# amazon-science/siam-mot

Hardware: AMD Instinct MI355X
Metric: frame-pairs/sec at 720p, 30 active tracks; EMM xcorr HBM GB/s vs peak (higher is better)
Workload: dtype f32 (towers and correlation: fp16x2 operands on MFMA, fp32 accumulate, fp32-equivalent error); 1 GPU; EMM tracker-head frame pair (EMM.forward + EMM.extract_cache) on DLA-34-FPN 720p FPN maps (net input 704x1280, C=128, 5 levels), 30 tracks, one stream per GPU; hot path only: backbone / RPN / box head / solver are outside the timed region; tracks=30, channels=128, rz=15, rx=30, feature_sets=8, feature_bytes_rotated=307281920

## Files before the change

siam-mot_amd/csrc/common.hip:

```cpp
#include "smot_common.h"
#include <mutex>
#include <vector>
#include "knobs.h"
#include <stdlib.h>
#include <string.h>

namespace smot {

static thread_local char g_err[512] = {0};

void set_error(const char* fmt, ...) {
    va_list ap;
    va_start(ap, fmt);
    vsnprintf(g_err, sizeof(g_err), fmt, ap);
    va_end(ap);
}

static thread_local int g_feat_type = SMOT_FEAT_F32;
int feat_type() { return g_feat_type & ~SMOT_FEAT_CHANNELS_LAST; }
bool channels_last() { return (g_feat_type & SMOT_FEAT_CHANNELS_LAST) != 0; }
FeatTypeScope::FeatTypeScope(int ft) : prev(g_feat_type) { g_feat_type = ft; }
FeatTypeScope::~FeatTypeScope() { g_feat_type = prev; }
int check_feat_type(int ft, const char* who) {
    const int et = ft & ~SMOT_FEAT_CHANNELS_LAST;
// ... 3 lines not shown
    return SMOT_ERR_BAD_ARG;
}

}

extern "C" int smot_abi_version(void) { return SMOT_ABI_VERSION; }

extern "C" int smot_build_info(void) {
#ifdef SMOT_DEBUG
    return 1;
#else
    return 0;
#endif
}

#ifdef SMOT_DEBUG
namespace smot {
namespace {
struct KnobName {
    const char* name;
    int Knobs::*field;
};
const KnobName kKnobNames[] = {
    {"SMOT_NO_FUSE", &Knobs::no_fuse},           {"SMOT_ROI_GENERIC", &Knobs::roi_generic},
    {"SMOT_TOWER_DIRECT", &Knobs::tower_direct}, {"SMOT_TOWER_WIDE", &Knobs::tower_wide},
    {"SMOT_DECODE_SPLIT", &Knobs::decode_split}, {"SMOT_XCORR_VARIANT", &Knobs::xcorr_variant},
    {"SMOT_DECODE_2PASS", &Knobs::decode_two_pass}, {"SMOT_FUSED_GEN", &Knobs::fused_gen},
    {"SMOT_TOWER_OCT", &Knobs::tower_oct},
    {"SMOT_TOWER_BF3", &Knobs::tower_bf3},
    {"SMOT_FUSED_ORDER", &Knobs::fused_order},   {"SMOT_NO_HINT", &Knobs::no_hint},
    {"SMOT_FUSED_ABL", &Knobs::fused_abl},       {"SMOT_ANY_ORDER", &Knobs::any_order},
    {"SMOT_WINO_ABL", &Knobs::wino_abl},
    {"SMOT_TOWER_ABL", &Knobs::tower_abl},
};
int parse_knob(const char* name, const char* v) {
    if (strcmp(name, "SMOT_XCORR_VARIANT") == 0) {
        static const char* const names[] = {"default", "wave", "patch", "pk", "one", "mfma", "fill", "compute"};
        for (int i = 0; i < 8; ++i)
            if (strcmp(v, names[i]) == 0) return i;
    }
    return atoi(v);
}
Knobs read_env() {
    Knobs k;
    for (const KnobName& kn : kKnobNames) {
        const char* v = getenv(kn.name);
        if (v != nullptr && v[0] != 0) k.*(kn.field) = parse_knob(kn.name, v);
    }
    return k;
}
}
Knobs& knobs_mut() {
    static Knobs k = read_env();
    return k;
}
namespace {
struct KnobInit {
    KnobInit() { (void)knobs_mut(); }
} g_knob_init;
}
}

extern "C" int smot_debug_set_knob(const char* name, const char* value) {
    using namespace smot;
    SMOT_REQUIRE(name && value, "debug_set_knob: null argument");
    for (const KnobName& kn : kKnobNames)
// ... 179 lines not shown
```

siam-mot_amd/csrc/knobs.h:

```cpp
#pragma once

namespace smot {

enum XcorrVariant { XV_DEFAULT = 0, XV_WAVE, XV_PATCH, XV_PK, XV_ONE, XV_MFMA, XV_FILL, XV_COMPUTE };

struct Knobs {
    int no_fuse = 0;
    int roi_generic = 0;
    int tower_direct = 0;
    int tower_wide = 0;
    int decode_split = 0;
    int xcorr_variant = 0;
    int decode_two_pass = 0;
    int fused_gen = 0;
    int fused_order = 0;
    int no_hint = 0;
    int tower_oct = 0;
    int tower_bf3 = 1;
    int any_order = 0;
    int fused_abl = 0;
    int wino_abl = 0;
    int tower_abl = 0;
};

#ifdef SMOT_DEBUG
Knobs& knobs_mut();
inline const Knobs& knobs() { return knobs_mut(); }
bool launch_xcorr_variant(int variant, const float* x, const float* z, float* out, int planes, hipStream_t st);
#else
inline constexpr Knobs knobs() { return Knobs{}; }
#endif

}
```

siam-mot_amd/csrc/sr_xcorr.hip:

```cpp
#include "roi_common.h"
#include "xcorr_patch2.h"
#include "xcorr_patch1.h"
#include "xcorr_f16x2.h"
#include "knobs.h"
#include <type_traits>
namespace smot { int launch_plane_absmax(const float* resp, int planes, int hw, float* pm, hipStream_t st); }

namespace smot {

constexpr int FX_CH = 8;

struct SrOut {
    float* sr;
    float pad, half_e, two_e, min_wh;
    long long* trace;
    int abl;
    const int* n_valid;
    int order;
    float* hint_out;
    const float* hint_in;
    int hint_extra;
    int plan_pad[SMOT_MAX_LEVELS];
    float* plane_max;
};
// ... 380 lines not shown
    constexpr bool BATCHED = true;
    constexpr int NCH = FX_CH;
    constexpr bool P2 = false;
    constexpr bool NHWC = true;
#include "sr_xcorr_fused9_body.h"
}

}


namespace smot {
constexpr int FX_ORDER_DEFAULT = 1;
static inline int fused_order() {
    const int k = knobs().fused_order;
    return k == 0 ? FX_ORDER_DEFAULT : (k == 4 ? 0 : k);
}
static inline bool order_hint_rois(int N, bool consumer) {
    if (knobs().fused_gen == 2 || knobs().no_hint >= (consumer ? 1 : 2)) return false;
    return N >= 2 && N <= 256 && fused_order() == 1;
}
template <int RX, bool XCORR, int MM>
static void launch_fused_half(dim3 grid, hipStream_t st, const LevelParams& P, int C, const float* rois, const float* boxes,
                              const float* z, float* resp, float* out, int32_t* levels_out, const SrOut& S,
                              const ImageRows* I) {
    SMOT_HALF_TYPES(
        if (I != nullptr) {
            SMOT_LAUNCH((sr_xcorr_fused9_half_batched_kernel<FT, RX, 15, 2, XCORR, MM>), grid, dim3(512), 0, st, P, C, rois,
                        boxes, z, resp, out, levels_out, S, *I);
        } else {
            SMOT_LAUNCH((sr_xcorr_fused9_half_kernel<FT, RX, 15, 2, XCORR, MM>), grid, dim3(512), 0, st, P, C, rois, boxes, z,
                        resp, out, levels_out, S);
        })
}
static inline bool half_maps() { return feat_type() != SMOT_FEAT_F32; }

template <int RX, bool XCORR, int MM>
static void launch_fused_nhwc(dim3 grid, hipStream_t st, const LevelParams& P, int C, const float* rois, const float* boxes,
                              const float* z, float* resp, float* out, int32_t* levels_out, const SrOut& S,
                              const ImageRows* I) {
    ImageRows one;
    if (I == nullptr) {
        one.num_images = 1;
        one.row_start[0] = 0;
        for (int b = 1; b <= SMOT_MAX_IMAGES; ++b) one.row_start[b] = (int)grid.x;
        I = &one;
    }
    if (feat_type() == SMOT_FEAT_F32) {
        SMOT_LAUNCH((sr_xcorr_fused9_nhwc_kernel<float, RX, 15, 2, XCORR, MM>), grid, dim3(512), 0, st, P, C, rois, boxes, z,
                    resp, out, levels_out, S, *I);
    } else {
        SMOT_HALF_TYPES(SMOT_LAUNCH((sr_xcorr_fused9_nhwc_kernel<FT, RX, 15, 2, XCORR, MM>), grid, dim3(512), 0, st, P, C,
                                    rois, boxes, z, resp, out, levels_out, S, *I))
    }
}
static void launch_pool_nhwc(int out_size, dim3 grid, hipStream_t st, const LevelParams& P, int C, const float* rois,
                             const float* boxes, float* out, int32_t* levels_out, const SrOut& S, const ImageRows* I) {
    if (out_size == 30) launch_fused_nhwc<30, false, 0>(grid, st, P, C, rois, boxes, nullptr, nullptr, out, levels_out, S, I);
    else if (out_size == 7) launch_fused_nhwc<7, false, 0>(grid, st, P, C, rois, boxes, nullptr, nullptr, out, levels_out, S, I);
    else launch_fused_nhwc<15, false, 0>(grid, st, P, C, rois, boxes, nullptr, nullptr, out, levels_out, S, I);
}

template <int RX, bool XCORR>
static void launch_fused(dim3 grid, hipStream_t st, const LevelParams& P, int C, const float* rois, const float* boxes,
                         const float* z, float* resp, float* out, int32_t* levels_out, const SrOut& S) {
    if (channels_last()) {
        launch_fused_nhwc<RX, XCORR, (RX == 30 && XCORR) ? 1 : 0>(grid, st, P, C, rois, boxes, z, resp, out, levels_out, S, nullptr);
// ... 6 lines not shown
#ifdef SMOT_DEBUG
    if (knobs().fused_gen == 2 && S.n_valid == nullptr) {
        hipLaunchKernelGGL((sr_xcorr_fused8_kernel<RX, 15, 2, XCORR>), grid, dim3(512), 0, st, P, C, rois, boxes, z, resp,
                           out, levels_out, S);
        return;
    }
#endif
    if constexpr (RX == 30 && XCORR) {
#ifdef SMOT_DEBUG
        if (knobs().fused_abl == 8 || knobs().fused_abl == 9) {
            SMOT_LAUNCH((sr_xcorr_fused9_kernel<RX, 15, 2, XCORR>), grid, dim3(512), knobs().fused_abl == 9 ? 26000 : 0, st, P, C, rois,
                        boxes, z, resp, out, levels_out, S);
            return;
        }
#endif
#ifdef SMOT_DEBUG
        if (knobs().fused_abl == 10) {
            SMOT_LAUNCH((sr_xcorr_fused9_kernel<RX, 15, 2, XCORR, FX_CH, false, 2>), grid, dim3(512), 0, st, P, C, rois, boxes, z,
                        resp, out, levels_out, S);
            return;
        }
#endif
        SMOT_LAUNCH((sr_xcorr_fused9_kernel<RX, 15, 2, XCORR, FX_CH, false, 1>), grid, dim3(512), 0, st, P, C, rois, boxes, z,
                    resp, out, levels_out, S);
    } else {
        SMOT_LAUNCH((sr_xcorr_fused9_kernel<RX, 15, 2, XCORR>), grid, dim3(512), 0, st, P, C, rois, boxes, z, resp, out,
                    levels_out, S);
    }
}

int launch_roi_pool_separable(const LevelParams& P, int C, const float* rois, const float* level_boxes, int R,
                              int out_size, float* out, int32_t* levels_out, hipStream_t st) {
    dim3 grid(R, (C + FX_CH - 1) / FX_CH);
    SrOut none = {nullptr, 0.f, 0.f, 0.f, 0.f, g_trace, 0, nullptr, fused_order(), nullptr, nullptr, 0};
    if (channels_last()) {
        launch_pool_nhwc(out_size, grid, st, P, C, rois, level_boxes, out, levels_out, none, nullptr);
    } else if (out_size == 30) {
        launch_fused<30, false>(grid, st, P, C, rois, level_boxes, nullptr, nullptr, out, levels_out, none);
    } else if (out_size == 7 && half_maps()) {
        launch_fused_half<7, false, 0>(grid, st, P, C, rois, level_boxes, nullptr, nullptr, out, levels_out, none, nullptr);
    } else if (out_size == 7) {
        SMOT_LAUNCH((sr_xcorr_fused9_kernel<7, 15, 2, false>), grid, dim3(512), 0, st, P, C, rois, level_boxes,
                    (const float*)nullptr, (float*)nullptr, out, levels_out, none);
    } else {
        launch_fused<15, false>(grid, st, P, C, rois, level_boxes, nullptr, nullptr, out, levels_out, none);
    }
    return check_launch("roi_pool_separable");
}

int launch_extract_cache(const float* const* feats, const int* heights, const int* widths, const float* scales,
                         int num_levels, int C, const float* boxes, int N, int rz, float pad_pixels, float half_e,
                         float two_e, float min_wh, float* templates, float* sr, const int* n_valid, float* order_hint,
                         hipStream_t st, int hint_extra_rows) {
    LevelParams P;
    const int rc = fill_level_params(&P, feats, heights, widths, nullptr, scales, num_levels, "emm_extract_cache", C);
    if (rc) return rc;
    SMOT_REQUIRE(boxes && templates && sr, "emm_extract_cache: null pointer");
    if (!order_hint_rois(N, false) || rz != 15) order_hint = nullptr;
    SMOT_REQUIRE(order_hint == nullptr || ((((uintptr_t)order_hint) & 31) == 0 && (((uintptr_t)boxes) & 15) == 0),
                 "emm_extract_cache: the order hint must be 32-byte aligned (and the boxes 16-byte aligned)");
    dim3 grid(N, (C + FX_CH - 1) / FX_CH + (order_hint != nullptr ? 1 : 0));
    SrOut S = {sr, pad_pixels, half_e, two_e, min_wh, g_trace, 0, n_valid, fused_order(), order_hint, nullptr,
               n_valid != nullptr ? hint_extra_rows : 0};
    for (int l = 0; l < num_levels && l < SMOT_MAX_LEVELS; ++l) S.plan_pad[l] = (int)(pad_pixels * scales[l]);
    if (channels_last()) {
        launch_pool_nhwc(rz, grid, st, P, C, boxes, boxes, templates, nullptr, S, nullptr);
    } else if (rz == 7 && half_maps()) {
        launch_fused_half<7, false, 0>(grid, st, P, C, boxes, boxes, nullptr, nullptr, templates, nullptr, S, nullptr);
    } else if (rz == 7) {
        SMOT_LAUNCH((sr_xcorr_fused9_kernel<7, 15, 2, false>), grid, dim3(512), 0, st, P, C, boxes, boxes, (const float*)nullptr,
                    (float*)nullptr, templates, (int32_t*)nullptr, S);
    } else {
        launch_fused<15, false>(grid, st, P, C, boxes, boxes, nullptr, nullptr, templates, nullptr, S);
    }
    return check_launch("emm_extract_cache");
}

int launch_roi_pool_separable_batched(const LevelParams& P, int C, const float* rois, const float* level_boxes, int R,
                                      int out_size, float* out, hipStream_t st, const ImageRows& I) {
    dim3 grid(R, (C + FX_CH - 1) / FX_CH);
    SrOut none = {nullptr, 0.f, 0.f, 0.f, 0.f, g_trace, 0, nullptr, fused_order(), nullptr, nullptr, 0};
    if (channels_last()) {
        launch_pool_nhwc(out_size, grid, st, P, C, rois, level_boxes, out, nullptr, none, &I);
    } else if (half_maps()) {
        if (out_size == 30) launch_fused_half<30, false, 0>(grid, st, P, C, rois, level_boxes, nullptr, nullptr, out, nullptr, none, &I);
        else if (out_size == 7) launch_fused_half<7, false, 0>(grid, st, P, C, rois, level_boxes, nullptr, nullptr, out, nullptr, none, &I);
        else launch_fused_half<15, false, 0>(grid, st, P, C, rois, level_boxes, nullptr, nullptr, out, nullptr, none, &I);
    } else if (out_size == 30) {
        SMOT_LAUNCH((sr_xcorr_fused9_batched_kernel<30, 15, 2, false>), grid, dim3(512), 0, st, P, C, rois, level_boxes,
                    (const float*)nullptr, (float*)nullptr, out, (int32_t*)nullptr, none, I);
    } else if (out_size == 7) {
        SMOT_LAUNCH((sr_xcorr_fused9_batched_kernel<7, 15, 2, false>), grid, dim3(512), 0, st, P, C, rois, level_boxes,
                    (const float*)nullptr, (float*)nullptr, out, (int32_t*)nullptr, none, I);
    } else {
        SMOT_LAUNCH((sr_xcorr_fused9_batched_kernel<15, 15, 2, false>), grid, dim3(512), 0, st, P, C, rois, level_boxes,
                    (const float*)nullptr, (float*)nullptr, out, (int32_t*)nullptr, none, I);
    }
    return check_launch("roi_pool_separable_batched");
}

int launch_extract_cache_batched(const float* const* feats, const int* heights, const int* widths, const float* scales,
                                 int num_levels, int C, const float* boxes, int N, int rz, float pad_pixels, float half_e,
                                 float two_e, float min_wh, float* templates, float* sr, float* order_hint, hipStream_t st,
                                 const ImageRows& I) {
    LevelParams P;
    const int rc = fill_level_params(&P, feats, heights, widths, nullptr, scales, num_levels, "emm_extract_cache_batched", C);
    if (rc) return rc;
    SMOT_REQUIRE(boxes && templates && sr, "emm_extract_cache_batched: null pointer");
    if (!order_hint_rois(N, false) || rz != 15) order_hint = nullptr;
    SMOT_REQUIRE(order_hint == nullptr || ((((uintptr_t)order_hint) & 31) == 0 && (((uintptr_t)boxes) & 15) == 0),
                 "emm_extract_cache_batched: the order hint must be 32-byte aligned (and the boxes 16-byte aligned)");
    dim3 grid(N, (C + FX_CH - 1) / FX_CH + (order_hint != nullptr ? 1 : 0));
    SrOut S = {sr, pad_pixels, half_e, two_e, min_wh, g_trace, 0, nullptr, fused_order(), order_hint, nullptr, 0};
    for (int l = 0; l < num_levels && l < SMOT_MAX_LEVELS; ++l) S.plan_pad[l] = (int)(pad_pixels * scales[l]);
    if (channels_last()) {
        launch_pool_nhwc(rz, grid, st, P, C, boxes, boxes, templates, nullptr, S, &I);
    } else if (half_maps()) {
        if (rz == 7) launch_fused_half<7, false, 0>(grid, st, P, C, boxes, boxes, nullptr, nullptr, templates, nullptr, S, &I);
        else launch_fused_half<15, false, 0>(grid, st, P, C, boxes, boxes, nullptr, nullptr, templates, nullptr, S, &I);
    } else if (rz == 7) {
        SMOT_LAUNCH((sr_xcorr_fused9_batched_kernel<7, 15, 2, false>), grid, dim3(512), 0, st, P, C, boxes, boxes,
                    (const float*)nullptr, (float*)nullptr, templates, (int32_t*)nullptr, S, I);
    } else {
        SMOT_LAUNCH((sr_xcorr_fused9_batched_kernel<15, 15, 2, false>), grid, dim3(512), 0, st, P, C, boxes, boxes,
                    (const float*)nullptr, (float*)nullptr, templates, (int32_t*)nullptr, S, I);
    }
    return check_launch("emm_extract_cache_batched");
}

int sr_xcorr_fused_batched_impl(const float* const* feats, const int* heights, const int* widths, const int* pad_cells,
                                const float* scales, int num_levels, int C, const float* boxes, const float* sr,
                                const float* templates, int N, float* resp, const float* order_hint, hipStream_t st,
                                const int** hint_status, float* plane_max, const ImageRows& I) {
    LevelParams P;
    const int rc = fill_level_params(&P, feats, heights, widths, pad_cells, scales, num_levels, "sr_xcorr_fused_batched", C);
    if (rc) return rc;
    if (!order_hint_rois(N, true)) order_hint = nullptr;
    if (hint_status != nullptr)
        *hint_status = order_hint != nullptr ? reinterpret_cast<const int*>(order_hint) + HINT_STATUS : nullptr;
    SMOT_REQUIRE(order_hint == nullptr || (((uintptr_t)order_hint) & 31) == 0,
                 "sr_xcorr_fused_batched: the order hint must be 32-byte aligned");
    dim3 grid(N, (C + FX_CH - 1) / FX_CH);
    SrOut none = {nullptr, 0.f, 0.f, 0.f, 0.f, g_trace, 0, nullptr, fused_order(), nullptr, order_hint, 0};
    none.plane_max = plane_max;
    timer_mark(0, 0, st);
    if (channels_last())
// ... 137 lines not shown
```

siam-mot_amd/csrc/sr_xcorr_fused9_body.h:

```cpp
    constexpr int HO = XCORR ? RX - RZ + 1 : 16;
    constexpr int NS = RX * G;
    constexpr int XS = P2 ? XP2_XS : (MM == 2 ? XL_XS : XP1_XS), XP = P2 ? XP2_XP : (MM == 2 ? 30 * XL_XS : 32 * XP1_XS), ZS = XP1_ZS,
                  ZP = MM == 1 ? XH_TZ_FLOATS : (MM == 2 ? XL_TZ_FLOATS : RZ * XP1_ZS);
    static_assert(MM == 0 || (XCORR && !P2 && RX == 30 && RZ == 15), "the matrix-pipe correlation is the 30 / 15 head's");
    static_assert(MM != 2 || ((XP * 4) % 128 == 0 && ((2 * XP + 2 * ZP) * 4) % 128 == 0), "lean layout: 128-byte aligned plane images");
    constexpr int RH = (RX + 1) / 2;
    static_assert((!XCORR || RX - RZ + 1 == 16) && RX <= 32 && G == 2 && RX * XS <= XP && 2 * RH * G <= 64,
                  "specialised for pooled sizes <= 32, g = 2 (and the 30/15/16 correlation geometry)");
    __shared__ __attribute__((aligned(128))) float sm[(NCH / 2) * (2 * XP + 2 * ZP)];
    __shared__ __attribute__((aligned(16))) int4 tab[2][64 + 2 * RH * G];
    __shared__ int wbound[4];

    const int tid = threadIdx.x;
    const int lane = tid & 63;
    const int wave = __builtin_amdgcn_readfirstlane(tid >> 6);
    const long long t_start = S.trace ? (long long)__builtin_amdgcn_s_memtime() : 0ll;
    const int ka_h = P.H[0], ka_w = P.W[0], ka_p = P.pad[0];
    const float ka_s = P.scale[0];
    const unsigned long long ka_f = reinterpret_cast<unsigned long long>(P.feat[0]);
#define SMOT_KA_USE() asm volatile("" ::"s"(ka_h), "s"(ka_w), "s"(ka_p), "s"(ka_s), "s"(ka_f))
    int ka_i[6] = {0, 0, 0, 0, 0, 0};
    if constexpr (BATCHED) {
        ka_i[0] = I.num_images;
#pragma unroll
        for (int k = 1; k < 6; ++k) ka_i[k] = I.row_start[min(16 * k - 1, SMOT_MAX_IMAGES)];
    }
#ifdef SMOT_DEBUG
    if (S.abl >= 100 && (int)(blockIdx.y * gridDim.x + blockIdx.x) >= 256) {
        for (int d = 0; d < S.abl - 100; ++d) __builtin_amdgcn_s_sleep(8);
    }
#endif
    int n_assigned, cg_assigned, lvl_assigned = 0;
    float4 roi_assigned = make_float4(0.f, 0.f, 0.f, 0.f);
    int grid_row = blockIdx.y, grid_rows = gridDim.y;
    if constexpr (!XCORR) {
        if (S.hint_out != nullptr) {
            if (grid_row == 0) {
                fx_write_hint<30, G>(P, boxes, S, gridDim.x, blockIdx.x, wave, lane);
                return;
            }
            grid_row -= 1;
            grid_rows -= 1;
        }
    }
// ... 64 lines not shown
        S.sr[n * 4 + 2] = o.z;
        S.sr[n * 4 + 3] = o.w;
    }
    const int H = P.H[lvl], W = P.W[lvl], pad = P.pad[lvl];
    const float scale = P.scale[lvl];
    const float x1 = mul_rn(roi[0], scale), y1 = mul_rn(roi[1], scale);
    const float x2 = mul_rn(roi[2], scale), y2 = mul_rn(roi[3], scale);
    const float bin_h = div_rn(fmaxf(sub_rn(y2, y1), 1.0f), (float)RX);
    const float bin_w = div_rn(fmaxf(sub_rn(x2, x1), 1.0f), (float)RX);
    FX_TRACE(6)
    constexpr int nplanes = NCH;
    const int c0 = cgrp * NCH;
    const bool owns = (wave < nplanes && c0 + wave < C);
    const int plane = n * C + c0 + wave;
    constexpr int NZ = XCORR ? (RZ * RZ + 63) / 64 : 1;
    float zreg[NZ];
    float zq[4] = {0.0f, 0.0f, 0.0f, 0.0f}, isz = 1.0f;
    if constexpr (MM != 0) {
        if (owns) xh_template_load(z + (size_t)plane * (RZ * RZ), lane, zq);
    } else if (XCORR && owns) {
        const float* __restrict__ zg = z + (size_t)plane * (RZ * RZ);
#pragma unroll
        for (int t = 0; t < NZ; ++t) zreg[t] = zg[min(lane + 64 * t, RZ * RZ - 1)];
    }

    const bool hent = XCORR && RX == 30 && k_assigned >= 0 && g8[4] == pad && g8[5] == H && g8[6] == W &&
                      g8[7] == __float_as_int(scale);
    const int hb[4] = {g8[0], g8[1], g8[2], g8[3]};
    const bool fast = !NHWC && MM == 1 && hent && hb[3] - hb[2] + 1 <= 64
#ifdef SMOT_DEBUG
                      && S.abl != 3 && S.abl != 12
#endif
        ;
    if (fast) {
    } else if (wave < 2 && hent) {
        tab[wave][lane] = tab_early;
        if (lane < 2 * RH * G) tab[wave][64 + lane] = make_int4(0, 0, 0, 0);
    } else if (wave < 2) {
        int lo = 0, hi = 0;
        float wl = 0.0f, wh = 0.0f;
        if (lane < NS) {
            if (wave == 0) {
                axis_sample(y1, bin_h, G, lane, H, pad, &lo, &hi, &wl, &wh);
            } else {
                axis_sample(x1, bin_w, G, lane, W, pad, &lo, &hi, &wl, &wh);
            }
        }
        int mn = 0x7fffffff, mx = -1;
        const unsigned long long m = __ballot(wl != 0.0f || wh != 0.0f);
        if (m != 0ull) {
            mn = __builtin_amdgcn_readlane((wl != 0.0f) ? lo : hi, __ffsll((long long)m) - 1);
            mx = __builtin_amdgcn_readlane((wh != 0.0f) ? hi : lo, 63 - __clzll((long long)m));
        }
        const int rl = (wl != 0.0f) ? lo : mn, rh = (wh != 0.0f) ? hi : mn;
        int4 e;
        if (wave == 0) {
            e.x = (int)((unsigned)(rl * W) * 4u);
            e.y = (int)((unsigned)(rh * W) * 4u);
        } else {
            e.x = (wl != 0.0f) ? lo - mn : 0;
            e.y = (wh != 0.0f) ? hi - mn : 0;
        }
        e.z = __float_as_int(wl);
        e.w = __float_as_int(wh);
        tab[wave][lane] = e;
        if (lane < 2 * RH * G) tab[wave][64 + lane] = make_int4(0, 0, 0, 0);
        if (lane == 0) {
            wbound[2 * wave] = mn;
            wbound[2 * wave + 1] = mx;
        }
    }
    FX_TRACE(7)
    if (!fast) __syncthreads();
    const int ymin = hent ? hb[0] : wbound[0], ymax = hent ? hb[1] : wbound[1];
    const int xmin = hent ? hb[2] : wbound[2], xmax = hent ? hb[3] : wbound[3];
    if (ymax < ymin || xmax < xmin) {
        if (owns) {
            if (XCORR) {
                for (int e = lane; e < HO * HO; e += 64) resp[(size_t)plane * HO * HO + e] = 0.0f;
                if (S.plane_max != nullptr && lane == 0) S.plane_max[plane] = 0.0f;
            }
            if (x_debug != nullptr)
                for (int e = lane; e < RX * RX; e += 64) x_debug[(size_t)plane * RX * RX + e] = 0.0f;
        }
        return;
    }
    const int ww = xmax - xmin + 1;
    FX_TRACE(1)

    if constexpr (MM != 0) {
    } else if (XCORR && owns) {
        float* zs = sm + (wave >> 1) * (2 * XP + 2 * ZP) + 2 * XP + (wave & 1) * ZP;
#pragma unroll
        for (int t = 0; t < NZ; ++t) {
            const int e = lane + 64 * t;
            if (e < RZ * RZ) {
                const int u = e / RZ;
                zs[u * ZS + (e - u * RZ)] = zreg[t];
            }
        }
    }
    FX_TRACE(2)

    const FT* __restrict__ fbase = reinterpret_cast<const FT*>(P.feat[lvl]);
    if constexpr (BATCHED) fbase += (size_t)img * ((size_t)C * H * W);
    const unsigned plane_bytes = (unsigned)(H * W) * (unsigned)sizeof(FT);
    constexpr int ROW_SHIFT = sizeof(FT) == 2 ? 1 : 0;
    auto pool = [&](auto pair_tag, auto chunk_tag, auto x2_tag, auto rows_tag) {
        constexpr bool PAIR = decltype(pair_tag)::value;
        constexpr bool CHUNKED = decltype(chunk_tag)::value;
        constexpr bool X2 = decltype(x2_tag)::value;
        constexpr int ROWS = decltype(rows_tag)::value;
        constexpr int NV = X2 ? 2 : 1;
        static_assert(!X2 || (PAIR && !CHUNKED), "two columns per lane is a form of the plane-pair mode");
        const int half = PAIR ? (lane >> 5) : 0;
        const int col = PAIR ? (lane & 31) : lane;
        const int pw = col < RX ? col : 0;
        const int pl0 = PAIR ? 2 * (wave >> 1) : wave;
        const bool has0 = (c0 + pl0 < C);
        const bool has1 = PAIR && (c0 + pl0 + 1 < C);
        if (!has0) return;
        const bool mine = PAIR ? (half == 0 || has1) : true;
        const unsigned lane_plane = (PAIR && half == 1 && has1) ? plane_bytes : 0u;
        float* xdst = sm + ((pl0 + half) >> 1) * (2 * XP + 2 * ZP) + ((pl0 + half) & 1) * XP;
        const FT* pbase = fbase + (size_t)(c0 + pl0) * H * W;
        unsigned long long pa = reinterpret_cast<unsigned long long>(pbase);
        const unsigned pa_lo = __builtin_amdgcn_readfirstlane((unsigned)pa);
        const unsigned pa_hi = __builtin_amdgcn_readfirstlane((unsigned)(pa >> 32));
        const auto rsrc = __builtin_amdgcn_make_buffer_rsrc(
            reinterpret_cast<void*>(((unsigned long long)pa_hi << 32) | pa_lo), 0, 0x7fffffff, 0x00020000);
        int sxl[G], sxh[G];
        float hxw[G], lxw[G];
#pragma unroll
        for (int ix = 0; ix < G; ++ix) {
            const int4 e = fast ? xe_early[ix] : tab[1][pw * G + ix];
            sxl[ix] = e.x;
            sxh[ix] = e.y;
            hxw[ix] = __int_as_float(e.z);
            lxw[ix] = __int_as_float(e.w);
        }
        const int row0 = PAIR ? (wave & 1) * RH : 0;
        const int nrows = PAIR ? RH : RX;
        const int nchunk = CHUNKED ? (ww + 63) >> 6 : 1;
        if constexpr (X2 && MM == 1) {
            constexpr int GR = (ROWS + 1) / 2, SW = 64;
            static_assert(RH % ROWS == 0 && GR * SW <= ROWS * XS, "full batches; staging fits a batch's own rows");
            const int wcol = min(2 * col, ww - 2);
            const unsigned voff = (unsigned)(xmin + wcol) * (unsigned)sizeof(FT) + lane_plane;
            typename fx_pair<FT>::type vl[ROWS][G], vh[ROWS][G];
            int4 ye = fast ? ye_early : tab[0][min(lane + row0 * G, 63 + 2 * RH * G)];
            ye.x = (int)((unsigned)ye.x >> ROW_SHIFT);
            ye.y = (int)((unsigned)ye.y >> ROW_SHIFT);
            int yoff = 0;
#define SMOT_FX_ISSUE()                                                                                             \
            _Pragma("unroll") for (int b = 0; b < ROWS; ++b)                                                        \
                _Pragma("unroll") for (int iy = 0; iy < G; ++iy) {                                                  \
                    vl[b][iy] = fx_load2<FT>(rsrc, voff, __builtin_amdgcn_readlane(ye.x, yoff + b * G + iy));         \
                    vh[b][iy] = fx_load2<FT>(rsrc, voff, __builtin_amdgcn_readlane(ye.y, yoff + b * G + iy));         \
                }
            SMOT_FX_ISSUE()
            __builtin_amdgcn_sched_barrier(0);
            if (owns) {
                unsigned char* tzw = reinterpret_cast<unsigned char*>(sm + (wave >> 1) * (2 * XP + 2 * ZP) + 2 * XP + (wave & 1) * ZP);
                isz = xh_template_store(zq, tzw, lane);
            }
            __builtin_amdgcn_sched_barrier(0);
#pragma unroll 1
            for (int r0 = row0; r0 < row0 + nrows; r0 += ROWS) {
                const float wl = __int_as_float(ye.z), wh = __int_as_float(ye.w);
                float cs[ROWS][NV];
#pragma unroll
                for (int b = 0; b < ROWS; ++b)
// ... 27 lines not shown
                    for (int b = g0; b < g0 + GR && b < ROWS; ++b)
#pragma unroll
                        for (int k = 0; k < NV; ++k) stage[(b - g0) * SW + wcol + k] = cs[b][k];
                    float p[GR][G][2];
#pragma unroll
                    for (int b = g0; b < g0 + GR && b < ROWS; ++b)
#pragma unroll
                        for (int ix = 0; ix < G; ++ix) {
                            p[b - g0][ix][0] = stage[(b - g0) * SW + sxl[ix]];
                            p[b - g0][ix][1] = stage[(b - g0) * SW + sxh[ix]];
                        }
                    __builtin_amdgcn_sched_barrier(0);
#pragma unroll
                    for (int b = g0; b < g0 + GR && b < ROWS; ++b)
#pragma unroll
                        for (int ix = 0; ix < G; ++ix) {
                            acc[b] = fmaf(hxw[ix], p[b - g0][ix][0], ix == 0 ? 0.0f : acc[b]);
                            acc[b] = fmaf(lxw[ix], p[b - g0][ix][1], acc[b]);
                        }
                    __builtin_amdgcn_sched_barrier(0);
                }
#pragma unroll
                for (int b = 0; b < ROWS; ++b) {
                    const int ph = r0 + b;
                    if (col < RX && ph < row0 + nrows && ph < RX && mine) xdst[ph * XS + col] = acc[b] * (1.0f / (float)(G * G));
                }
            }
#undef SMOT_FX_ISSUE
            return;
        }
#pragma unroll 1
        for (int r0 = row0; r0 < row0 + nrows; r0 += ROWS) {
            const int4 ye = (fast && PAIR && !CHUNKED) ? ye_early : tab[0][min(lane + r0 * G, 63 + 2 * RH * G)];
            const unsigned ol = (unsigned)ye.x >> ROW_SHIFT, oh = (unsigned)ye.y >> ROW_SHIFT;
            const float wl = __int_as_float(ye.z), wh = __int_as_float(ye.w);
            float acc[ROWS];
            if (CHUNKED) {
#pragma unroll
                for (int b = 0; b < ROWS; ++b) acc[b] = 0.0f;
            }
#pragma unroll 1
            for (int ch = 0; ch < nchunk; ++ch) {
                const int cbase = ch << 6;
                const int wcol = CHUNKED ? min(cbase + col, ww - 1) : (X2 ? min(2 * col, ww - 2) : min(col, ww - 1));
                const unsigned voff = (unsigned)(xmin + wcol) * (unsigned)sizeof(FT) + lane_plane;
                float v[ROWS][G][2][NV];
#pragma unroll
                for (int b = 0; b < ROWS; ++b)
#pragma unroll
                    for (int iy = 0; iy < G; ++iy) {
                        const int e = b * G + iy;
                        if constexpr (X2) {
                            const auto l2 = fx_load2<FT>(rsrc, voff, __builtin_amdgcn_readlane((int)ol, e));
                            const auto h2 = fx_load2<FT>(rsrc, voff, __builtin_amdgcn_readlane((int)oh, e));
                            v[b][iy][0][0] = fx_pair_elem<FT>(l2, 0);
                            v[b][iy][0][NV - 1] = fx_pair_elem<FT>(l2, 1);
                            v[b][iy][1][0] = fx_pair_elem<FT>(h2, 0);
                            v[b][iy][1][NV - 1] = fx_pair_elem<FT>(h2, 1);
                        } else {
                            v[b][iy][0][0] = fx_load1<FT>(rsrc, voff, __builtin_amdgcn_readlane((int)ol, e));
                            v[b][iy][1][0] = fx_load1<FT>(rsrc, voff, __builtin_amdgcn_readlane((int)oh, e));
                        }
                    }
                __builtin_amdgcn_sched_barrier(0);
                if constexpr (MM != 0) {
                    if (r0 == row0 && ch == 0 && owns) {
                        unsigned char* tzw = reinterpret_cast<unsigned char*>(sm + (wave >> 1) * (2 * XP + 2 * ZP) + 2 * XP + (wave & 1) * ZP);
                        isz = MM == 2 ? xl_template_store(zq, tzw, lane) : xh_template_store(zq, tzw, lane);
                    }
                    __builtin_amdgcn_sched_barrier(0);
                }
                float cs[ROWS][NV];
#pragma unroll
                for (int b = 0; b < ROWS; ++b)
#pragma unroll
                    for (int k = 0; k < NV; ++k) {
                        float c_ = 0.0f;
#pragma unroll
                        for (int iy = 0; iy < G; ++iy) {
                            const int e = b * G + iy;
                            c_ = fmaf(rl_f(wl, e), v[b][iy][0][k], c_);
                            c_ = fmaf(rl_f(wh, e), v[b][iy][1][k], c_);
                        }
                        cs[b][k] = c_;
                    }
                __builtin_amdgcn_sched_barrier(0);
                constexpr int GR = ((P2 || MM == 2) && X2) ? 3 : (ROWS + 1) / 2;
                if constexpr (!CHUNKED) {
                    constexpr int SW = (X2 || !PAIR) ? 64 : 32;
                    static_assert(GR * SW <= (RH - (RH / ROWS) * ROWS == 0 ? ROWS : RH - (RH / ROWS) * ROWS) * XS,
                                  "staging fits the image rows of the wave's LAST batch");
                    float* stage = xdst + r0 * XS;
#pragma unroll
                    for (int g0 = 0; g0 < ROWS; g0 += GR) {
#pragma unroll
                        for (int b = g0; b < g0 + GR && b < ROWS; ++b)
#pragma unroll
                            for (int k = 0; k < NV; ++k) stage[(b - g0) * SW + wcol + k] = cs[b][k];
                        float p[GR][G][2];
#pragma unroll
                        for (int b = g0; b < g0 + GR && b < ROWS; ++b)
#pragma unroll
                            for (int ix = 0; ix < G; ++ix) {
                                p[b - g0][ix][0] = stage[(b - g0) * SW + sxl[ix]];
                                p[b - g0][ix][1] = stage[(b - g0) * SW + sxh[ix]];
                            }
                        __builtin_amdgcn_sched_barrier(0);
#pragma unroll
                        for (int b = g0; b < g0 + GR && b < ROWS; ++b)
#pragma unroll
                            for (int ix = 0; ix < G; ++ix) {
                                acc[b] = fmaf(hxw[ix], p[b - g0][ix][0], ix == 0 ? 0.0f : acc[b]);
                                acc[b] = fmaf(lxw[ix], p[b - g0][ix][1], acc[b]);
// ... 5 lines not shown
                    bool inl[G], inh[G];
#pragma unroll
                    for (int ix = 0; ix < G; ++ix) {
                        const int tl = sxl[ix] - cbase, th = sxh[ix] - cbase;
                        inl[ix] = (unsigned)tl < 64u;
                        inh[ix] = (unsigned)th < 64u;
                        al[ix] = (tl & 63) << 2;
                        ah[ix] = (th & 63) << 2;
                    }
#pragma unroll
                    for (int g0 = 0; g0 < ROWS; g0 += GR) {
                        float p[GR][G][2];
#pragma unroll
                        for (int b = g0; b < g0 + GR && b < ROWS; ++b)
#pragma unroll
                            for (int ix = 0; ix < G; ++ix) {
                                p[b - g0][ix][0] = __int_as_float(__builtin_amdgcn_ds_bpermute(al[ix], __float_as_int(cs[b][0])));
                                p[b - g0][ix][1] = __int_as_float(__builtin_amdgcn_ds_bpermute(ah[ix], __float_as_int(cs[b][0])));
                            }
                        __builtin_amdgcn_sched_barrier(0);
#pragma unroll
                        for (int b = g0; b < g0 + GR && b < ROWS; ++b)
#pragma unroll
                            for (int ix = 0; ix < G; ++ix) {
                                acc[b] = inl[ix] ? fmaf(hxw[ix], p[b - g0][ix][0], acc[b]) : acc[b];
                                acc[b] = inh[ix] ? fmaf(lxw[ix], p[b - g0][ix][1], acc[b]) : acc[b];
                            }
                    }
                }
            }
#pragma unroll
            for (int b = 0; b < ROWS; ++b) {
                const int ph = r0 + b;
                if (col < RX && ph < row0 + nrows && ph < RX && mine) xdst[ph * XS + col] = acc[b] * (1.0f / (float)(G * G));
            }
        }
    };
    if constexpr (NHWC) {
#include "sr_pool_nhwc_stage.h"
    } else
    if (ww <= 32) {
        pool(std::true_type{}, std::false_type{}, std::false_type{}, std::integral_constant<int, RH>{});
#ifdef SMOT_DEBUG
    } else if (ww <= 64 && S.abl == 3 && MM != 2) {
        if constexpr (MM != 2) pool(std::false_type{}, std::false_type{}, std::false_type{}, std::integral_constant<int, RH>{});
#endif
    } else if (ww <= 64) {
        if constexpr (MM == 1) pool(std::true_type{}, std::false_type{}, std::true_type{}, std::integral_constant<int, RH / 3>{});
        else pool(std::true_type{}, std::false_type{}, std::true_type{}, std::integral_constant<int, (RH + 1) / 2>{});
    } else {
        pool(std::false_type{}, std::true_type{}, std::false_type{}, std::integral_constant<int, (RH + 2) / 3>{});
    }
    FX_TRACE(3)
    __syncthreads();
    if (x_debug != nullptr && owns) {
        const float* xs = sm + (wave >> 1) * (2 * XP + 2 * ZP) + (wave & 1) * XP;
        for (int e = lane; e < RX * RX; e += 64) {
            const int r = e / RX;
            x_debug[(size_t)plane * RX * RX + e] = xs[r * XS + (e - r * RX)];
        }
    }
    if constexpr (XCORR) {
#ifdef SMOT_DEBUG
        if (S.abl == 2) return;
#endif
        if constexpr (P2) {
            if (wave < nplanes / 2 && c0 + 2 * wave < C) {
                const float* xs2 = sm + wave * (2 * XP + 2 * ZP);
                xcorr_patch2_compute<RX, RZ, 0>(xs2, xs2 + 2 * XP, lane, resp, n * C + c0 + 2 * wave, n * C + min(C, c0 + NCH));
            }
        } else if (owns) {
            float* xs1 = sm + (wave >> 1) * (2 * XP + 2 * ZP) + (wave & 1) * XP;
            const float* zs1 = sm + (wave >> 1) * (2 * XP + 2 * ZP) + 2 * XP + (wave & 1) * ZP;
            if constexpr (MM == 1) xh_correlate<RX, RZ>(xs1, reinterpret_cast<const unsigned char*>(zs1), isz, lane, resp, plane, S.plane_max);
            else if constexpr (MM == 2) xl_correlate<RX, RZ>(xs1, reinterpret_cast<const unsigned char*>(zs1), isz, lane, resp, plane, S.plane_max);
            else xcorr_patch1_compute<RX, RZ, true>(xs1, zs1, lane, resp, plane, S.plane_max);
        }
    }
    FX_TRACE(4)
#undef FX_TRACE
```

siam-mot_amd/ops.py:

```python
import contextlib
import ctypes
import struct
import weakref
import os

import torch

_HERE = os.path.dirname(os.path.abspath(__file__))
LIB_PATH = os.path.join(_HERE, "csrc", "libsmot_emm.so")
DEBUG_LIB_PATH = os.path.join(_HERE, "csrc", "libsmot_emm_debug.so")
ABI_VERSION = 14
UP_SCALE = 16


_lib = None
_c_float_p = ctypes.POINTER(ctypes.c_float)
_vp = ctypes.c_void_p
_i = ctypes.c_int
_f = ctypes.c_float

_SIGNATURES = {
    "smot_abi_version": (ctypes.c_int, []),
    "smot_build_info": (ctypes.c_int, []),
    "smot_last_error": (ctypes.c_char_p, []),
# ... 82 lines not shown
    "smot_debug_sr_xcorr_fused_hint_fwd": (ctypes.c_int, [_vp, _vp, _vp, _vp, _vp, _i, _i, _vp, _vp, _vp, _i, _vp, _vp, _vp]),
}
DEBUG_EXPORTED_SYMBOLS = tuple(_DEBUG_SIGNATURES.keys())


def load_library(path=None):
    global _lib
    if _lib is not None and path is None:
        return _lib
    path = path or LIB_PATH
    if not os.path.exists(path):
        raise RuntimeError(
            "siammot_amd: HIP library %s not found — build it with `python siam-mot_amd/build.py` "
            "(hipcc --offload-arch=gfx950).  There is no CPU fallback." % path)
    _lib = _open(path, _SIGNATURES)
    return _lib


def _open(path, signatures):
    lib = ctypes.CDLL(path)
    for name, (res, args) in signatures.items():
        fn = getattr(lib, name)
        fn.restype = res
        fn.argtypes = args
    if lib.smot_abi_version() != ABI_VERSION:
        raise RuntimeError("siammot_amd: %s has ABI %d, host layer expects %d"
                           % (path, lib.smot_abi_version(), ABI_VERSION))
    return lib


_KNOB_DEFAULTS = {"SMOT_NO_FUSE": "0", "SMOT_ROI_GENERIC": "0", "SMOT_TOWER_DIRECT": "0", "SMOT_TOWER_WIDE": "0",
                  "SMOT_DECODE_SPLIT": "0", "SMOT_XCORR_VARIANT": "default", "SMOT_DECODE_2PASS": "0",
                  "SMOT_FUSED_GEN": "0", "SMOT_TOWER_OCT": "0", "SMOT_TOWER_BF3": "1", "SMOT_FUSED_ORDER": "0", "SMOT_NO_HINT": "0", "SMOT_FUSED_ABL": "0",
                  "SMOT_ANY_ORDER": "0",
                  "SMOT_WINO_ABL": "0",
                  "SMOT_TOWER_ABL": "0"}


@contextlib.contextmanager
def debug_library(**knobs):
    global _lib
    if not os.path.exists(DEBUG_LIB_PATH):
        raise RuntimeError("siammot_amd: measurement library %s not built (python siam-mot_amd/build.py)" % DEBUG_LIB_PATH)
    load_library()
    dbg = _open(DEBUG_LIB_PATH, dict(_SIGNATURES, **_DEBUG_SIGNATURES))
    if not (dbg.smot_build_info() & 1):
        raise RuntimeError("siammot_amd: %s is not a measurement build" % DEBUG_LIB_PATH)
    prev, _lib = _lib, dbg

    def set_all(values):
        for k, v in values.items():
            if dbg.smot_debug_set_knob(k.encode(), str(v).encode()) != 0:
                raise RuntimeError("siammot_amd: " + dbg.smot_last_error().decode("utf-8", "replace"))
    try:
        set_all(_KNOB_DEFAULTS)
        set_all(knobs)
        _hint_floats.clear()
        yield dbg
    finally:
        set_all(_KNOB_DEFAULTS)
        _lib = prev
        _hint_floats.clear()


def _check(rc, what):
    if rc != 0:
        msg = _lib.smot_last_error().decode("utf-8", "replace")
# ... 1290 lines not shown
```

Baseline: 18400 frame-pairs/s.

## Add lean pool-only extraction path with register tables and direct global stores

For the non-xcorr, NCHW pooling instantiation (template extraction), each wave now computes its y/x sampling entries in registers and reads them by lane through bpermute and readlane. This replaces the shared-memory table build, its barrier, and the reduction of bounds through shared memory. Pooled outputs are written straight to global memory instead of being staged in LDS and copied out after a __syncthreads. The aim is to cut barriers and LDS traffic in the short extraction kernel. The cost is scattered, stride-RX global stores and more cross-lane shuffles; a debug knob keeps the old path, and a trace script is added.

```diff
diff --git a/measure/debug/extract_trace.py b/measure/debug/extract_trace.py
--- /dev/null
+++ b/measure/debug/extract_trace.py
@@ -0,0 +1,51 @@
+import json, os, sys
+import numpy as np, torch
+sys.path.insert(0, os.path.join(os.path.dirname(__file__), "..", ".."))
+import bench
+import siammot_amd.ops as ops
+dev = torch.device("cuda:0")
+ops.load_library()
+scales = (0.25, 0.125, 0.0625, 0.03125)
+args = sys.argv[1:]
+split = args.index("--") if "--" in args else len(args)
+counts = [int(a) for a in args[:split]] or [30]
+variants = [dict(kv.split("=") for kv in v.split(",")) for v in args[split + 1:]] or [{}]
+PHASES = ("assign", "level+bins", "table build", "table barrier", "pool", "tail: barrier + store")
+
+
+def stats(x):
+    return {"mean": round(float(x.mean())), "p90": round(float(np.percentile(x, 90))), "max": int(x.max())}
+
+
+for n in counts:
+    boxes = bench.synthetic_boxes(n, (1280, 704)).to(dev)
+    feats = [bench.synthetic_features(k, dev) for k in range(4)]
+    rows = (feats[0][0].shape[1] + 7) // 8
+    for var in variants:
+        with ops.debug_library(**var) as dbg:
+            def run(i, tr=None):
+                dbg.smot_debug_trace(ops._ptr(tr) if tr is not None else None)
+                out = ops.emm_extract_cache(feats[i % 4], boxes, 15, scales, 2, 512.0, 1.0, 0.0, hint=True)
+                dbg.smot_debug_trace(None)
+                return out
+            for i in range(20): run(i)
+            torch.cuda.synchronize()
+            e0, e1 = torch.cuda.Event(enable_timing=True), torch.cuda.Event(enable_timing=True)
+            e0.record()
+            for i in range(200): run(i)
+            e1.record(); torch.cuda.synchronize()
+            us = e0.elapsed_time(e1) / 200 * 1e3
+            ts = []
+            for i in range(8):
+                tr = torch.zeros(n * rows * 8, dtype=torch.int64, device=dev)
+                run(i, tr); torch.cuda.synchronize()
+                ts.append(tr.view(n, rows, 8).cpu().numpy().astype(np.float64))
+        t = np.concatenate(ts, 0)
+        ran = (t[:, :, 4] > 0) & (t[:, :, 0] > 0)
+        chain = t[:, :, [0, 5, 6, 7, 1, 3, 4]]
+        d = np.diff(chain, axis=2)[ran]
+        total = (t[:, :, 4] - t[:, :, 0])[ran]
+        print(json.dumps({"kernel": "extraction 15x15 with hint row", "tracks": n, "variant": var,
+                          "back_to_back_us_per_launch": round(us, 2), "workgroups_traced": int(ran.sum()),
+                          "phase_ticks": {p: stats(d[:, k]) for k, p in enumerate(PHASES)},
+                          "workgroup_total_ticks": stats(total)}), flush=True)
diff --git a/siam-mot_amd/csrc/common.hip b/siam-mot_amd/csrc/common.hip
--- a/siam-mot_amd/csrc/common.hip
+++ b/siam-mot_amd/csrc/common.hip
@@ -59,6 +59,7 @@
     {"SMOT_FUSED_ABL", &Knobs::fused_abl},       {"SMOT_ANY_ORDER", &Knobs::any_order},
     {"SMOT_WINO_ABL", &Knobs::wino_abl},
     {"SMOT_TOWER_ABL", &Knobs::tower_abl},
+    {"SMOT_EXTRACT_OLD", &Knobs::extract_old},
 };
 int parse_knob(const char* name, const char* v) {
     if (strcmp(name, "SMOT_XCORR_VARIANT") == 0) {
diff --git a/siam-mot_amd/csrc/knobs.h b/siam-mot_amd/csrc/knobs.h
--- a/siam-mot_amd/csrc/knobs.h
+++ b/siam-mot_amd/csrc/knobs.h
@@ -17,6 +17,7 @@
     int no_hint = 0;
     int tower_oct = 0;
     int tower_bf3 = 1;
+    int extract_old = 0;
     int any_order = 0;
     int fused_abl = 0;
     int wino_abl = 0;
diff --git a/siam-mot_amd/csrc/sr_xcorr.hip b/siam-mot_amd/csrc/sr_xcorr.hip
--- a/siam-mot_amd/csrc/sr_xcorr.hip
+++ b/siam-mot_amd/csrc/sr_xcorr.hip
@@ -436,6 +436,7 @@
                         resp, out, levels_out, S);
         })
 }
+static inline int pool_abl() { return knobs().extract_old ? 20 : 0; }
 static inline bool half_maps() { return feat_type() != SMOT_FEAT_F32; }
 
 template <int RX, bool XCORR, int MM>
@@ -508,7 +509,7 @@
 int launch_roi_pool_separable(const LevelParams& P, int C, const float* rois, const float* level_boxes, int R,
                               int out_size, float* out, int32_t* levels_out, hipStream_t st) {
     dim3 grid(R, (C + FX_CH - 1) / FX_CH);
-    SrOut none = {nullptr, 0.f, 0.f, 0.f, 0.f, g_trace, 0, nullptr, fused_order(), nullptr, nullptr, 0};
+    SrOut none = {nullptr, 0.f, 0.f, 0.f, 0.f, g_trace, pool_abl(), nullptr, fused_order(), nullptr, nullptr, 0};
     if (channels_last()) {
         launch_pool_nhwc(out_size, grid, st, P, C, rois, level_boxes, out, levels_out, none, nullptr);
     } else if (out_size == 30) {
@@ -536,7 +537,7 @@
     SMOT_REQUIRE(order_hint == nullptr || ((((uintptr_t)order_hint) & 31) == 0 && (((uintptr_t)boxes) & 15) == 0),
                  "emm_extract_cache: the order hint must be 32-byte aligned (and the boxes 16-byte aligned)");
     dim3 grid(N, (C + FX_CH - 1) / FX_CH + (order_hint != nullptr ? 1 : 0));
-    SrOut S = {sr, pad_pixels, half_e, two_e, min_wh, g_trace, 0, n_valid, fused_order(), order_hint, nullptr,
+    SrOut S = {sr, pad_pixels, half_e, two_e, min_wh, g_trace, pool_abl(), n_valid, fused_order(), order_hint, nullptr,
                n_valid != nullptr ? hint_extra_rows : 0};
     for (int l = 0; l < num_levels && l < SMOT_MAX_LEVELS; ++l) S.plan_pad[l] = (int)(pad_pixels * scales[l]);
     if (channels_last()) {
@@ -555,7 +556,7 @@
 int launch_roi_pool_separable_batched(const LevelParams& P, int C, const float* rois, const float* level_boxes, int R,
                                       int out_size, float* out, hipStream_t st, const ImageRows& I) {
     dim3 grid(R, (C + FX_CH - 1) / FX_CH);
-    SrOut none = {nullptr, 0.f, 0.f, 0.f, 0.f, g_trace, 0, nullptr, fused_order(), nullptr, nullptr, 0};
+    SrOut none = {nullptr, 0.f, 0.f, 0.f, 0.f, g_trace, pool_abl(), nullptr, fused_order(), nullptr, nullptr, 0};
     if (channels_last()) {
         launch_pool_nhwc(out_size, grid, st, P, C, rois, level_boxes, out, nullptr, none, &I);
     } else if (half_maps()) {
@@ -587,7 +588,7 @@
     SMOT_REQUIRE(order_hint == nullptr || ((((uintptr_t)order_hint) & 31) == 0 && (((uintptr_t)boxes) & 15) == 0),
                  "emm_extract_cache_batched: the order hint must be 32-byte aligned (and the boxes 16-byte aligned)");
     dim3 grid(N, (C + FX_CH - 1) / FX_CH + (order_hint != nullptr ? 1 : 0));
-    SrOut S = {sr, pad_pixels, half_e, two_e, min_wh, g_trace, 0, nullptr, fused_order(), order_hint, nullptr, 0};
+    SrOut S = {sr, pad_pixels, half_e, two_e, min_wh, g_trace, pool_abl(), nullptr, fused_order(), order_hint, nullptr, 0};
     for (int l = 0; l < num_levels && l < SMOT_MAX_LEVELS; ++l) S.plan_pad[l] = (int)(pad_pixels * scales[l]);
     if (channels_last()) {
         launch_pool_nhwc(rz, grid, st, P, C, boxes, boxes, templates, nullptr, S, &I);
diff --git a/siam-mot_amd/csrc/sr_xcorr_fused9_body.h b/siam-mot_amd/csrc/sr_xcorr_fused9_body.h
--- a/siam-mot_amd/csrc/sr_xcorr_fused9_body.h
+++ b/siam-mot_amd/csrc/sr_xcorr_fused9_body.h
@@ -10,6 +10,12 @@
     __shared__ __attribute__((aligned(128))) float sm[(NCH / 2) * (2 * XP + 2 * ZP)];
     __shared__ __attribute__((aligned(16))) int4 tab[2][64 + 2 * RH * G];
     __shared__ int wbound[4];
+    constexpr bool LEAN_C = !XCORR && !NHWC, LEAN_T = LEAN_C && NS <= 32;
+#ifdef SMOT_DEBUG
+    const bool lean = LEAN_C && S.abl != 20, lean_t = LEAN_T && lean;
+#else
+    constexpr bool lean = LEAN_C, lean_t = LEAN_T;
+#endif
 
     const int tid = threadIdx.x;
     const int lane = tid & 63;
@@ -140,7 +146,44 @@
                       && S.abl != 3 && S.abl != 12
 #endif
         ;
-    if (fast) {
+    constexpr int XL = 32;
+    constexpr int LR2 = (RH + 1) / 2, LR3 = (RH + 2) / 3;
+    static_assert(!LEAN_T || (2 * RH * G <= XL && (RH + (RH + LR2 - 1) / LR2 * LR2) * G <= XL && (RX + LR3 - 1) / LR3 * LR3 * G <= XL),
+                  "lean: a batch's y entries are read out of the wave's own table by lane");
+    int4 yxt = make_int4(0, 0, 0, 0);
+    int lb[4] = {0, -1, 0, -1};
+    if constexpr (LEAN_T) {
+        if (lean_t) {
+            auto bounds = [&](unsigned long long m, int lo, int hi, float wl, float wh, int* mn, int* mx) {
+                *mn = 0x7fffffff;
+                *mx = -1;
+                if (m != 0ull) {
+                    *mn = __builtin_amdgcn_readlane((wl != 0.0f) ? lo : hi, __ffsll((long long)m) - 1);
+                    *mx = __builtin_amdgcn_readlane((wh != 0.0f) ? hi : lo, 63 - __clzll((long long)m));
+                }
+            };
+            const bool xl = lane >= XL;
+            const int s = lane & (XL - 1);
+            int lo = 0, hi = 0;
+            float wl = 0.0f, wh = 0.0f;
+            if (s < NS) axis_sample(xl ? x1 : y1, xl ? bin_w : bin_h, G, s, xl ? W : H, pad, &lo, &hi, &wl, &wh);
+            const unsigned long long m = __ballot(wl != 0.0f || wh != 0.0f);
+            bounds(m & 0xffffffffull, lo, hi, wl, wh, &lb[0], &lb[1]);
+            bounds(m & ~0xffffffffull, lo, hi, wl, wh, &lb[2], &lb[3]);
+            const int mn = xl ? lb[2] : lb[0];
+            const int rl = (wl != 0.0f) ? lo : mn, rh = (wh != 0.0f) ? hi : mn;
+            yxt.x = xl ? ((wl != 0.0f) ? lo - mn : 0) : (int)((unsigned)(rl * W) * 4u);
+            yxt.y = xl ? ((wh != 0.0f) ? hi - mn : 0) : (int)((unsigned)(rh * W) * 4u);
+            yxt.z = __float_as_int(wl);
+            yxt.w = __float_as_int(wh);
+        }
+    }
+    auto lean_xe = [&](int idx) {
+        const int a = (idx + XL) << 2;
+        return make_int4(__builtin_amdgcn_ds_bpermute(a, yxt.x), __builtin_amdgcn_ds_bpermute(a, yxt.y),
+                         __builtin_amdgcn_ds_bpermute(a, yxt.z), __builtin_amdgcn_ds_bpermute(a, yxt.w));
+    };
+    if (fast || lean_t) {
     } else if (wave < 2 && hent) {
         tab[wave][lane] = tab_early;
         if (lane < 2 * RH * G) tab[wave][64 + lane] = make_int4(0, 0, 0, 0);
@@ -179,9 +222,9 @@
         }
     }
     FX_TRACE(7)
-    if (!fast) __syncthreads();
-    const int ymin = hent ? hb[0] : wbound[0], ymax = hent ? hb[1] : wbound[1];
-    const int xmin = hent ? hb[2] : wbound[2], xmax = hent ? hb[3] : wbound[3];
+    if (!fast && !lean_t) __syncthreads();
+    const int ymin = lean_t ? lb[0] : (hent ? hb[0] : wbound[0]), ymax = lean_t ? lb[1] : (hent ? hb[1] : wbound[1]);
+    const int xmin = lean_t ? lb[2] : (hent ? hb[2] : wbound[2]), xmax = lean_t ? lb[3] : (hent ? hb[3] : wbound[3]);
     if (ymax < ymin || xmax < xmin) {
         if (owns) {
             if (XCORR) {
@@ -231,6 +274,8 @@
         const bool mine = PAIR ? (half == 0 || has1) : true;
         const unsigned lane_plane = (PAIR && half == 1 && has1) ? plane_bytes : 0u;
         float* xdst = sm + ((pl0 + half) >> 1) * (2 * XP + 2 * ZP) + ((pl0 + half) & 1) * XP;
+        float* odst = nullptr;
+        if constexpr (LEAN_C) odst = x_debug + (size_t)(n * C + c0 + pl0 + half) * (RX * RX) + pw;
         const FT* pbase = fbase + (size_t)(c0 + pl0) * H * W;
         unsigned long long pa = reinterpret_cast<unsigned long long>(pbase);
         const unsigned pa_lo = __builtin_amdgcn_readfirstlane((unsigned)pa);
@@ -246,6 +291,18 @@
             sxh[ix] = e.y;
             hxw[ix] = __int_as_float(e.z);
             lxw[ix] = __int_as_float(e.w);
+        }
+        if constexpr (LEAN_T) {
+            if (lean_t) {
+#pragma unroll
+                for (int ix = 0; ix < G; ++ix) {
+                    const int4 e = lean_xe(pw * G + ix);
+                    sxl[ix] = e.x;
+                    sxh[ix] = e.y;
+                    hxw[ix] = __int_as_float(e.z);
+                    lxw[ix] = __int_as_float(e.w);
+                }
+            }
         }
         const int row0 = PAIR ? (wave & 1) * RH : 0;
         const int nrows = PAIR ? RH : RX;
@@ -339,8 +396,18 @@
 #pragma unroll 1
         for (int r0 = row0; r0 < row0 + nrows; r0 += ROWS) {
             const int4 ye = (fast && PAIR && !CHUNKED) ? ye_early : tab[0][min(lane + r0 * G, 63 + 2 * RH * G)];
-            const unsigned ol = (unsigned)ye.x >> ROW_SHIFT, oh = (unsigned)ye.y >> ROW_SHIFT;
-            const float wl = __int_as_float(ye.z), wh = __int_as_float(ye.w);
+            unsigned ol = (unsigned)ye.x >> ROW_SHIFT, oh = (unsigned)ye.y >> ROW_SHIFT;
+            float wl = __int_as_float(ye.z), wh = __int_as_float(ye.w);
+            int yb = 0;
+            if constexpr (LEAN_T) {
+                if (lean_t) {
+                    ol = (unsigned)yxt.x >> ROW_SHIFT;
+                    oh = (unsigned)yxt.y >> ROW_SHIFT;
+                    wl = __int_as_float(yxt.z);
+                    wh = __int_as_float(yxt.w);
+                    yb = r0 * G;
+                }
+            }
             float acc[ROWS];
             if (CHUNKED) {
 #pragma unroll
@@ -356,7 +423,7 @@
                 for (int b = 0; b < ROWS; ++b)
 #pragma unroll
                     for (int iy = 0; iy < G; ++iy) {
-                        const int e = b * G + iy;
+                        const int e = yb + b * G + iy;
                         if constexpr (X2) {
                             const auto l2 = fx_load2<FT>(rsrc, voff, __builtin_amdgcn_readlane((int)ol, e));
                             const auto h2 = fx_load2<FT>(rsrc, voff, __builtin_amdgcn_readlane((int)oh, e));
@@ -385,7 +452,7 @@
                         float c_ = 0.0f;
 #pragma unroll
                         for (int iy = 0; iy < G; ++iy) {
-                            const int e = b * G + iy;
+                            const int e = yb + b * G + iy;
                             c_ = fmaf(rl_f(wl, e), v[b][iy][0][k], c_);
                             c_ = fmaf(rl_f(wh, e), v[b][iy][1][k], c_);
                         }
@@ -457,7 +524,17 @@
 #pragma unroll
             for (int b = 0; b < ROWS; ++b) {
                 const int ph = r0 + b;
-                if (col < RX && ph < row0 + nrows && ph < RX && mine) xdst[ph * XS + col] = acc[b] * (1.0f / (float)(G * G));
+                if (col < RX && ph < row0 + nrows && ph < RX && mine) {
+                    if constexpr (LEAN_C) {
+                        if (lean) {
+                            if (x_debug != nullptr) odst[ph * RX] = acc[b] * (1.0f / (float)(G * G));
+                        } else {
+                            xdst[ph * XS + col] = acc[b] * (1.0f / (float)(G * G));
+                        }
+                    } else {
+                        xdst[ph * XS + col] = acc[b] * (1.0f / (float)(G * G));
+                    }
+                }
             }
         }
     };
@@ -477,6 +554,7 @@
         pool(std::false_type{}, std::true_type{}, std::false_type{}, std::integral_constant<int, (RH + 2) / 3>{});
     }
     FX_TRACE(3)
+    if (!lean) {
     __syncthreads();
     if (x_debug != nullptr && owns) {
         const float* xs = sm + (wave >> 1) * (2 * XP + 2 * ZP) + (wave & 1) * XP;
@@ -484,6 +562,7 @@
             const int r = e / RX;
             x_debug[(size_t)plane * RX * RX + e] = xs[r * XS + (e - r * RX)];
         }
+    }
     }
     if constexpr (XCORR) {
 #ifdef SMOT_DEBUG
diff --git a/siam-mot_amd/ops.py b/siam-mot_amd/ops.py
--- a/siam-mot_amd/ops.py
+++ b/siam-mot_amd/ops.py
@@ -138,7 +138,7 @@
 _KNOB_DEFAULTS = {"SMOT_NO_FUSE": "0", "SMOT_ROI_GENERIC": "0", "SMOT_TOWER_DIRECT": "0", "SMOT_TOWER_WIDE": "0",
                   "SMOT_DECODE_SPLIT": "0", "SMOT_XCORR_VARIANT": "default", "SMOT_DECODE_2PASS": "0",
                   "SMOT_FUSED_GEN": "0", "SMOT_TOWER_OCT": "0", "SMOT_TOWER_BF3": "1", "SMOT_FUSED_ORDER": "0", "SMOT_NO_HINT": "0", "SMOT_FUSED_ABL": "0",
-                  "SMOT_ANY_ORDER": "0",
+                  "SMOT_ANY_ORDER": "0", "SMOT_EXTRACT_OLD": "0",
                   "SMOT_WINO_ABL": "0",
                   "SMOT_TOWER_ABL": "0"}
 
```

New measurement: 18560 frame-pairs/s (median of 3 runs). No clear change (+0.9%).
